# PufferAI/PufferLib

Hardware: NVIDIA H100
Metric: agent-steps/sec (env step + PPO rollout/update hot path) (higher is better)
Workload: dtype f32 (env state int32; policy GEMMs tf32 like the reference)

## Files before the change

pufferlib_b200/csrc/mlp_update.cu:

```cuda
#include <cuda.h>
#include <stdlib.h>

#include "pb_common.cuh"
#include "tma.cuh"
#include "wgmma.cuh"

namespace {

constexpr int TILE_M = 64, HID = 128, FEAT = 128, NO = 8;
constexpr int KBLK = 32;
constexpr int W_KBLK_BYTES = HID * KBLK * 4;
constexpr int X_KBLK_BYTES = TILE_M * KBLK * 4;
constexpr int X_TILE_BYTES = 4 * X_KBLK_BYTES;
constexpr int G_KBLK_BYTES = HID * 32 * 4;
constexpr int NSTAGE = 3;
constexpr int THREADS = 256;
constexpr int SM_W = 0;
constexpr int SM_X = 4 * W_KBLK_BYTES;
constexpr int SM_G = SM_X + NSTAGE * X_TILE_BYTES;
constexpr int SM_WH = SM_G + 2 * G_KBLK_BYTES;
constexpr int SM_BE = SM_WH + NO * HID * 4;
constexpr int SM_OUT = SM_BE + HID * 4;
constexpr int SM_DO = SM_OUT + 2 * TILE_M * NO * 4;
constexpr int SM_RED = SM_DO + TILE_M * NO * 4;
constexpr int SM_BAR = SM_RED + 8 * NO * 4;
constexpr int SMEM_TOTAL = SM_BAR + 64;
constexpr int TAIL = NO * HID + HID + NO;
static_assert(SMEM_TOTAL <= 227 * 1024, "shared memory budget (227 KiB per block on sm_90)");

struct FusedParams {
    const int64_t* actions;
    const float* old_logprobs;
    const float* adv;
    const float* returns;
    const float* old_values;
    const float* adv_norm;
    int64_t row_slab_stride;
    int64_t m;
    int64_t slab_rows;
    int64_t slab_stride_rows;
    int tiles_per_slab, n_tiles;
    int n_act;
    float clip, vclip, vf_coef, ent_coef;
    int clip_vloss;
    float* part_dw;
    float* part_tail;
    double* stats;
    float* dpre_out;
    float* dbg_hidden;
    float* dbg_dpre;
    float* dbg_dout;
    const float* w_heads;
    const float* b_enc;
    const float* b_heads;
};

__device__ __forceinline__ void tma_load_2d(void* dst, const CUtensorMap* map, int c0, int c1, uint64_t* bar) {
    asm volatile(
        "cp.async.bulk.tensor.2d.shared::cluster.global.tile.mbarrier::complete_tx::bytes [%0], [%1, {%2, %3}], [%4];" ::"r"(
            smem_u32(dst)),
        "l"(reinterpret_cast<uint64_t>(map)), "r"(c0), "r"(c1), "r"(smem_u32(bar))
        : "memory");
}

__device__ __forceinline__ uint32_t to_tf32(float x) {
    uint32_t r;
    asm("cvt.rna.tf32.f32 %0, %1;" : "=r"(r) : "f"(x));
    return r;
}

__device__ __forceinline__ void mma_tf32(float (&c)[4], const uint32_t (&a)[4], uint32_t b0, uint32_t b1) {
    asm volatile("mma.sync.aligned.m16n8k8.row.col.f32.tf32.tf32.f32 {%0,%1,%2,%3}, {%4,%5,%6,%7}, {%8,%9}, {%0,%1,%2,%3};"
                 : "+f"(c[0]), "+f"(c[1]), "+f"(c[2]), "+f"(c[3])
                 : "r"(a[0]), "r"(a[1]), "r"(a[2]), "r"(a[3]), "r"(b0), "r"(b1));
}

__device__ __forceinline__ uint32_t g_off(int n, int l) {
    return (uint32_t)((l >> 5) * G_KBLK_BYTES + n * 128 + ((((l & 31) >> 2) ^ (n & 7)) << 4) + (l & 3) * 4);
}
__device__ __forceinline__ uint32_t x_off(int r, int f) {
    return (uint32_t)((f >> 5) * X_KBLK_BYTES + r * 128 + ((((f & 31) >> 2) ^ (r & 7)) << 4) + (f & 3) * 4);
}

struct RowStats { float pg, v, ent, okl, kl, clipped; };

__device__ __forceinline__ RowStats ppo_row_sub(float z_lo, float z_hi, int sub, int lane, const FusedParams& p, int act,
                                                float old_lp, float adv, float ret, float old_v, float& g_lo, float& g_hi) {
    const unsigned full = 0xffffffffu;
    const int n = p.n_act;
    const bool lo_ok = sub < n, hi_ok = sub + 4 < n;
    float mx = fmaxf(lo_ok ? z_lo : -INFINITY, hi_ok ? z_hi : -INFINITY);
    mx = fmaxf(mx, __shfl_xor_sync(full, mx, 1));
    mx = fmaxf(mx, __shfl_xor_sync(full, mx, 2));
    float sum = (lo_ok ? expf(z_lo - mx) : 0.f) + (hi_ok ? expf(z_hi - mx) : 0.f);
    sum += __shfl_xor_sync(full, sum, 1);
    sum += __shfl_xor_sync(full, sum, 2);
    const float lse = mx + logf(sum);
    const float nl_lo = z_lo - lse, nl_hi = z_hi - lse;
    const float pk_lo = lo_ok ? expf(nl_lo) : 0.f, pk_hi = hi_ok ? expf(nl_hi) : 0.f;
    float ent = -(lo_ok ? pk_lo * nl_lo : 0.f) - (hi_ok ? pk_hi * nl_hi : 0.f);
    ent += __shfl_xor_sync(full, ent, 1);
    ent += __shfl_xor_sync(full, ent, 2);
    const int a = act < 0 ? 0 : (act >= n ? n - 1 : act);
    const int base = lane & ~3;
    const float nl_a = __shfl_sync(full, (a >> 2) ? nl_hi : nl_lo, base | (a & 3));
    const float v_new = __shfl_sync(full, (n >> 2) ? z_hi : z_lo, base | (n & 3));
    const float logratio = nl_a - old_lp;
    const float ratio = expf(logratio);
    const float pg1 = -adv * ratio;
    const float rc = fminf(fmaxf(ratio, 1.f - p.clip), 1.f + p.clip);
    const float pg2 = -adv * rc;
    const float pg = fmaxf(pg1, pg2);
    const float in_range = (ratio >= 1.f - p.clip && ratio <= 1.f + p.clip) ? 1.f : 0.f;
    float g_ratio;
    if (pg1 > pg2) g_ratio = -adv;
    else if (pg1 < pg2) g_ratio = -adv * in_range;
    else g_ratio = 0.5f * (-adv) + 0.5f * (-adv * in_range);
    const float inv_m = 1.0f / (float)p.m;
    const float g_nlp = g_ratio * ratio * inv_m;
    const float dv = v_new - ret;
    float vl, g_v;
    if (p.clip_vloss) {
        const float d = v_new - old_v;
        const float dc = fminf(fmaxf(d, -p.vclip), p.vclip);
        const float vc = old_v + dc;
        const float vu = dv * dv, vcl = (vc - ret) * (vc - ret);
        vl = fmaxf(vu, vcl);
        const float v_in = (d >= -p.vclip && d <= p.vclip) ? 1.f : 0.f;
        const float gu = 2.f * dv, gc = 2.f * (vc - ret) * v_in;
        g_v = vu > vcl ? gu : (vu < vcl ? gc : 0.5f * (gu + gc));
    } else {
        vl = dv * dv;
        g_v = 2.f * dv;
    }
    const float gv_out = 0.5f * p.vf_coef * g_v * inv_m;
    const float g_ent = p.ent_coef * inv_m;
    g_lo = lo_ok ? g_nlp * ((sub == a ? 1.f : 0.f) - pk_lo) + g_ent * pk_lo * (nl_lo + ent) : 0.f;
    g_hi = hi_ok ? g_nlp * ((sub + 4 == a ? 1.f : 0.f) - pk_hi) + g_ent * pk_hi * (nl_hi + ent) : 0.f;
    if (sub == n) g_lo = gv_out;
    if (sub + 4 == n) g_hi = gv_out;
    RowStats s;
    s.pg = pg; s.v = vl; s.ent = ent; s.okl = -logratio; s.kl = (ratio - 1.f) - logratio;
    s.clipped = fabsf(ratio - 1.f) > p.clip ? 1.f : 0.f;
    return s;
}

template <bool TF32_EPI, bool DW_KERNEL>
__global__ void __launch_bounds__(THREADS, 1)
k_mlp_update(const __grid_constant__ CUtensorMap map_x, const __grid_constant__ CUtensorMap map_w, const FusedParams p) {
    extern __shared__ __align__(1024) uint8_t smem[];
    uint64_t* w_full = reinterpret_cast<uint64_t*>(smem + SM_BAR);
    uint64_t* x_full = w_full + 1;
    float* wh = reinterpret_cast<float*>(smem + SM_WH);
    const float* be = reinterpret_cast<const float*>(smem + SM_BE);
    float* outp = reinterpret_cast<float*>(smem + SM_OUT);
    float* dos = reinterpret_cast<float*>(smem + SM_DO);
    float* red = reinterpret_cast<float*>(smem + SM_RED);
    uint8_t* gbuf = smem + SM_G;
    const int tid = threadIdx.x, warp = tid >> 5, lane = tid & 31, g = lane >> 2, t = lane & 3;
    const int wg = warp >> 2, wq = warp & 3;
    const int n_my = (p.n_tiles - (int)blockIdx.x + (int)gridDim.x - 1) / (int)gridDim.x;

    auto issue = [&](int it) {
        const int tile = (int)blockIdx.x + it * (int)gridDim.x;
        const int64_t row0 = (int64_t)(tile / p.tiles_per_slab) * p.slab_stride_rows + (int64_t)(tile % p.tiles_per_slab) * TILE_M;
        const int s = it % NSTAGE;
        mbar_expect_tx(&x_full[s], X_TILE_BYTES);
        for (int kb = 0; kb < 4; ++kb)
            tma_load_2d(smem + SM_X + s * X_TILE_BYTES + kb * X_KBLK_BYTES, &map_x, kb * KBLK, (int)row0, &x_full[s]);
    };
    if (tid == 0) {
        mbar_init(w_full, 1);
        for (int s = 0; s < NSTAGE; ++s) mbar_init(&x_full[s], 1);
        mbar_fence_init();
    }
    for (int i = tid; i < NO * HID; i += THREADS) wh[i] = p.w_heads[i];
    if (tid < HID) reinterpret_cast<float*>(smem + SM_BE)[tid] = p.b_enc[tid];
    __syncthreads();
    if (tid == 0) {
        mbar_expect_tx(w_full, 4 * W_KBLK_BYTES);
        for (int kb = 0; kb < 4; ++kb) tma_load_2d(smem + SM_W + kb * W_KBLK_BYTES, &map_w, kb * KBLK, 0, w_full);
        for (int it = 0; it < NSTAGE && it < n_my; ++it) issue(it);
    }

    const int hr0 = 64 * wg + 16 * wq + g, hr1 = hr0 + 8;
    const int lr = tid >> 2, sub = tid & 3;
    const float bh_lo = p.b_heads[sub], bh_hi = p.b_heads[sub + 4];
    uint32_t hb[8][2], ga[4];
    float whr[2][NO];
    if (TF32_EPI) {
        const int hh = warp >> 2;
#pragma unroll
        for (int ks = 0; ks < 8; ++ks) {
            hb[ks][0] = to_tf32(wh[g * HID + 64 * hh + 8 * ks + t]);
            hb[ks][1] = to_tf32(wh[g * HID + 64 * hh + 8 * ks + t + 4]);
        }
        ga[0] = to_tf32(wh[t * HID + hr0]);
        ga[1] = to_tf32(wh[t * HID + hr1]);
        ga[2] = to_tf32(wh[(t + 4) * HID + hr0]);
        ga[3] = to_tf32(wh[(t + 4) * HID + hr1]);
    } else {
#pragma unroll
        for (int a = 0; a < NO; ++a) {
            whr[0][a] = wh[a * HID + hr0];
            whr[1][a] = wh[a * HID + hr1];
        }
    }

    float dwacc[64];
#pragma unroll
    for (int i = 0; i < 64; ++i) dwacc[i] = 0.f;
    float dwh[4] = {0.f, 0.f, 0.f, 0.f};
    float be_acc[2] = {0.f, 0.f};
    float bh_acc[2] = {0.f, 0.f};
    double st[6] = {0, 0, 0, 0, 0, 0};
    const float adv_mean = p.adv_norm ? p.adv_norm[0] : 0.f, adv_rstd = p.adv_norm ? p.adv_norm[1] : 1.f;
    const bool need_old_v = p.clip_vloss || !p.returns;
    const uint32_t w_addr = smem_u32(smem + SM_W), g_addr = smem_u32(gbuf);

    for (int it = 0; it < n_my; ++it) {
        const int s = it % NSTAGE;
        const int tile = (int)blockIdx.x + it * (int)gridDim.x;
        const int slab = tile / p.tiles_per_slab, tis = tile - slab * p.tiles_per_slab;
        const int64_t lrow0 = (int64_t)tis * TILE_M;
        const int rows_left = (int)(p.slab_rows - lrow0 < TILE_M ? p.slab_rows - lrow0 : TILE_M);
        const int64_t i0 = (int64_t)slab * p.slab_rows + lrow0;
        const bool valid = lr < rows_left;
        int act = 0;
        float old_lp = 0.f, adv = 0.f, ret = 0.f, old_v = 0.f;
        if (valid) {
            const int64_t ri = (int64_t)slab * p.row_slab_stride + lrow0 + lr;
            act = (int)p.actions[ri];
            old_lp = p.old_logprobs[ri];
            adv = p.adv[ri];
            if (need_old_v) old_v = p.old_values[ri];
            if (p.returns) ret = p.returns[ri];
        }
        if (it == 0) mbar_wait(w_full, 0);
        mbar_wait(&x_full[s], (uint32_t)((it / NSTAGE) & 1));
        const uint8_t* xs = smem + SM_X + s * X_TILE_BYTES;
        const uint32_t x_addr = smem_u32(xs);

        float h[32];
#pragma unroll
        for (int i = 0; i < 32; ++i) h[i] = 0.f;
        wgmma_fence();
#pragma unroll
        for (int kb = 0; kb < 4; ++kb)
#pragma unroll
            for (int k = 0; k < 4; ++k)
                wgmma_m64n64k8_ss(h, wgmma_desc_sw128(w_addr + kb * W_KBLK_BYTES + wg * 8192 + k * 32),
                                  wgmma_desc_sw128(x_addr + kb * X_KBLK_BYTES + k * 32), (kb | k) ? 1 : 0);
        wgmma_commit();
        wgmma_wait<0>();
        wgmma_fence_acc(h);

        {
            const float b0 = be[hr0], b1 = be[hr1];
#pragma unroll
            for (int j = 0; j < 8; ++j) {
                h[4 * j] = fmaxf(h[4 * j] + b0, 0.f);
                h[4 * j + 1] = fmaxf(h[4 * j + 1] + b0, 0.f);
                h[4 * j + 2] = fmaxf(h[4 * j + 2] + b1, 0.f);
                h[4 * j + 3] = fmaxf(h[4 * j + 3] + b1, 0.f);
                const int l = 8 * j + 2 * t;
                *reinterpret_cast<float2*>(gbuf + g_off(hr0, l)) = make_float2(h[4 * j], h[4 * j + 1]);
                *reinterpret_cast<float2*>(gbuf + g_off(hr1, l)) = make_float2(h[4 * j + 2], h[4 * j + 3]);
                if (p.dbg_hidden) {
#pragma unroll
                    for (int e = 0; e < 4; ++e) {
                        const int le = l + (e & 1), he = (e & 2) ? hr1 : hr0;
                        if (le < rows_left) p.dbg_hidden[(i0 + le) * HID + he] = h[4 * j + e];
                    }
                }
            }
        }
        __syncthreads();

        if (TF32_EPI) {
            const int l0 = 16 * (warp & 3) + g, hh = warp >> 2;
            float c[4] = {0.f, 0.f, 0.f, 0.f};
#pragma unroll
            for (int ks = 0; ks < 8; ++ks) {
                const int n0 = 64 * hh + 8 * ks + t;
                const uint32_t a[4] = {*reinterpret_cast<const uint32_t*>(gbuf + g_off(n0, l0)),
                                       *reinterpret_cast<const uint32_t*>(gbuf + g_off(n0, l0 + 8)),
                                       *reinterpret_cast<const uint32_t*>(gbuf + g_off(n0 + 4, l0)),
                                       *reinterpret_cast<const uint32_t*>(gbuf + g_off(n0 + 4, l0 + 8))};
                mma_tf32(c, a, hb[ks][0], hb[ks][1]);
            }
            *reinterpret_cast<float2*>(outp + (hh * TILE_M + l0) * NO + 2 * t) = make_float2(c[0], c[1]);
            *reinterpret_cast<float2*>(outp + (hh * TILE_M + l0 + 8) * NO + 2 * t) = make_float2(c[2], c[3]);
        } else {
            const int l = tid & (TILE_M - 1), a0 = 2 * (tid >> 6);
            float o0 = 0.f, o1 = 0.f;
            if (a0 <= p.n_act) {
#pragma unroll 8
                for (int n = 0; n < HID; ++n) {
                    const float rh = *reinterpret_cast<const float*>(gbuf + g_off(n, l));
                    o0 = fmaf(rh, wh[a0 * HID + n], o0);
                    o1 = fmaf(rh, wh[(a0 + 1) * HID + n], o1);
                }
            }
            *reinterpret_cast<float2*>(outp + l * NO + a0) = make_float2(o0, o1);
        }
        __syncthreads();

        {
            float z_lo = bh_lo + outp[lr * NO + sub], z_hi = bh_hi + outp[lr * NO + sub + 4];
            if (TF32_EPI) {
                z_lo += outp[(TILE_M + lr) * NO + sub];
                z_hi += outp[(TILE_M + lr) * NO + sub + 4];
            }
            const float r_ = p.returns ? ret : adv + old_v;
            const float a_ = (adv - adv_mean) * adv_rstd;
            float g_lo, g_hi;
            const RowStats rs = ppo_row_sub(z_lo, z_hi, sub, lane, p, act, old_lp, a_, r_, old_v, g_lo, g_hi);
            if (!valid) g_lo = g_hi = 0.f;
            if (valid && sub == 0) {
                st[0] += rs.pg; st[1] += rs.v; st[2] += rs.ent; st[3] += rs.okl; st[4] += rs.kl; st[5] += rs.clipped;
            }
            bh_acc[0] += g_lo;
            bh_acc[1] += g_hi;
            dos[lr * NO + sub] = g_lo;
            dos[lr * NO + sub + 4] = g_hi;
            if (p.dbg_dout && valid) {
                p.dbg_dout[(i0 + lr) * 8 + sub] = g_lo;
                p.dbg_dout[(i0 + lr) * 8 + sub + 4] = g_hi;
            }
        }
        __syncthreads();

        float dp[32];
#pragma unroll
        for (int j = 0; j < 8; ++j) {
            if (TF32_EPI) {
                float c[4] = {0.f, 0.f, 0.f, 0.f};
                mma_tf32(c, ga, __float_as_uint(dos[(8 * j + g) * NO + t]), __float_as_uint(dos[(8 * j + g) * NO + t + 4]));
                dp[4 * j] = c[0]; dp[4 * j + 1] = c[1]; dp[4 * j + 2] = c[2]; dp[4 * j + 3] = c[3];
            } else {
                const int l = 8 * j + 2 * t;
                const float4 d0a = *reinterpret_cast<const float4*>(dos + l * NO), d0b = *reinterpret_cast<const float4*>(dos + l * NO + 4);
                const float4 d1a = *reinterpret_cast<const float4*>(dos + (l + 1) * NO), d1b = *reinterpret_cast<const float4*>(dos + (l + 1) * NO + 4);
                const float d0[8] = {d0a.x, d0a.y, d0a.z, d0a.w, d0b.x, d0b.y, d0b.z, d0b.w};
                const float d1[8] = {d1a.x, d1a.y, d1a.z, d1a.w, d1b.x, d1b.y, d1b.z, d1b.w};
                float s00 = 0.f, s01 = 0.f, s10 = 0.f, s11 = 0.f;
#pragma unroll
                for (int a = 0; a < NO; ++a) {
                    s00 = fmaf(d0[a], whr[0][a], s00);
                    s01 = fmaf(d1[a], whr[0][a], s01);
                    s10 = fmaf(d0[a], whr[1][a], s10);
                    s11 = fmaf(d1[a], whr[1][a], s11);
                }
                dp[4 * j] = s00; dp[4 * j + 1] = s01; dp[4 * j + 2] = s10; dp[4 * j + 3] = s11;
            }
#pragma unroll
            for (int e = 0; e < 4; ++e) dp[4 * j + e] = h[4 * j + e] > 0.f ? dp[4 * j + e] : 0.f;
            be_acc[0] += dp[4 * j] + dp[4 * j + 1];
            be_acc[1] += dp[4 * j + 2] + dp[4 * j + 3];
            const float b0 = dos[(8 * j + 2 * t) * NO + g], b1 = dos[(8 * j + 2 * t + 1) * NO + g];
            if (TF32_EPI) {
                const uint32_t a[4] = {__float_as_uint(h[4 * j]), __float_as_uint(h[4 * j + 2]), __float_as_uint(h[4 * j + 1]),
                                       __float_as_uint(h[4 * j + 3])};
                mma_tf32(dwh, a, __float_as_uint(b0), __float_as_uint(b1));
            } else {
                const uint32_t a[4] = {to_tf32(h[4 * j]), to_tf32(h[4 * j + 2]), to_tf32(h[4 * j + 1]), to_tf32(h[4 * j + 3])};
                mma_tf32(dwh, a, to_tf32(b0), to_tf32(b1));
            }
            const int l = 8 * j + 2 * t;
            if (p.dbg_dpre) {
#pragma unroll
                for (int e = 0; e < 4; ++e) {
                    const int le = l + (e & 1), he = (e & 2) ? hr1 : hr0;
                    if (le < rows_left) p.dbg_dpre[(i0 + le) * HID + he] = dp[4 * j + e];
                }
            }
            if (DW_KERNEL) {
                *reinterpret_cast<uint2*>(gbuf + g_off(hr0, l)) = make_uint2(to_tf32(dp[4 * j]), to_tf32(dp[4 * j + 1]));
                *reinterpret_cast<uint2*>(gbuf + g_off(hr1, l)) = make_uint2(to_tf32(dp[4 * j + 2]), to_tf32(dp[4 * j + 3]));
            } else {
                *reinterpret_cast<float2*>(gbuf + g_off(hr0, l)) = make_float2(dp[4 * j], dp[4 * j + 1]);
                *reinterpret_cast<float2*>(gbuf + g_off(hr1, l)) = make_float2(dp[4 * j + 2], dp[4 * j + 3]);
            }
        }

        if (DW_KERNEL) {
            fence_proxy_async_smem();
            __syncthreads();
            const int f0 = 64 * wg + 16 * wq + g;
            uint32_t xa[8][4];
#pragma unroll
            for (int ks = 0; ks < 8; ++ks) {
                const int r0 = 8 * ks + t;
                xa[ks][0] = to_tf32(*reinterpret_cast<const float*>(xs + x_off(r0, f0)));
                xa[ks][1] = to_tf32(*reinterpret_cast<const float*>(xs + x_off(r0, f0 + 8)));
                xa[ks][2] = to_tf32(*reinterpret_cast<const float*>(xs + x_off(r0 + 4, f0)));
                xa[ks][3] = to_tf32(*reinterpret_cast<const float*>(xs + x_off(r0 + 4, f0 + 8)));
            }
            wgmma_fence();
#pragma unroll
            for (int ks = 0; ks < 8; ++ks)
                wgmma_m64n128k8_rs(dwacc, xa[ks], wgmma_desc_sw128(g_addr + (ks >> 2) * G_KBLK_BYTES + (ks & 3) * 32), 1);
            wgmma_commit();
            wgmma_wait<0>();
            wgmma_fence_acc(dwacc);
#pragma unroll
            for (int ks = 0; ks < 8; ++ks)
#pragma unroll
                for (int i = 0; i < 4; ++i) asm volatile("" : "+r"(xa[ks][i])::"memory");
        } else {
            __syncthreads();
#pragma unroll
            for (int k = 0; k < TILE_M / 8; ++k) {
                const int l = 8 * warp + k;
                if (l < rows_left) {
                    const int n = 4 * lane;
                    const float4 v = make_float4(*reinterpret_cast<const float*>(gbuf + g_off(n, l)),
                                                 *reinterpret_cast<const float*>(gbuf + g_off(n + 1, l)),
                                                 *reinterpret_cast<const float*>(gbuf + g_off(n + 2, l)),
                                                 *reinterpret_cast<const float*>(gbuf + g_off(n + 3, l)));
                    __stcs(reinterpret_cast<float4*>(p.dpre_out + (i0 + l) * HID + n), v);
                }
            }
        }
        __syncthreads();
        if (tid == 0 && it + NSTAGE < n_my) {
            fence_proxy_async_smem();
            issue(it + NSTAGE);
        }
    }

    if (DW_KERNEL) {
        float* pd = p.part_dw + (int64_t)blockIdx.x * FEAT * HID;
        const int f0 = 64 * wg + 16 * wq + g;
#pragma unroll
        for (int j = 0; j < 16; ++j) {
            *reinterpret_cast<float2*>(pd + f0 * HID + 8 * j + 2 * t) = make_float2(dwacc[4 * j], dwacc[4 * j + 1]);
            *reinterpret_cast<float2*>(pd + (f0 + 8) * HID + 8 * j + 2 * t) = make_float2(dwacc[4 * j + 2], dwacc[4 * j + 3]);
        }
    }
    float* pt = p.part_tail + (int64_t)blockIdx.x * TAIL;
    pt[(2 * t) * HID + hr0] = dwh[0];
    pt[(2 * t + 1) * HID + hr0] = dwh[1];
    pt[(2 * t) * HID + hr1] = dwh[2];
    pt[(2 * t + 1) * HID + hr1] = dwh[3];
#pragma unroll
    for (int k = 0; k < 2; ++k) {
        be_acc[k] += __shfl_xor_sync(0xffffffffu, be_acc[k], 1);
        be_acc[k] += __shfl_xor_sync(0xffffffffu, be_acc[k], 2);
    }
    if (t == 0) {
        pt[NO * HID + hr0] = be_acc[0];
        pt[NO * HID + hr1] = be_acc[1];
    }
#pragma unroll
    for (int k = 0; k < 2; ++k)
#pragma unroll
        for (int off = 4; off < 32; off <<= 1) bh_acc[k] += __shfl_xor_sync(0xffffffffu, bh_acc[k], off);
    if (lane < 4) {
        red[warp * NO + lane] = bh_acc[0];
        red[warp * NO + lane + 4] = bh_acc[1];
    }
#pragma unroll
    for (int k = 0; k < 6; ++k) {
        double x = st[k];
#pragma unroll
        for (int off = 16; off > 0; off >>= 1) x += __shfl_xor_sync(0xffffffffu, x, off);
        if (lane == 0) atomicAdd(p.stats + k, x);
    }
    __syncthreads();
    if (tid < NO) {
        float v = 0.f;
        for (int w = 0; w < THREADS / 32; ++w) v += red[w * NO + tid];
        pt[NO * HID + HID + tid] = v;
    }
}

__global__ void __launch_bounds__(256) k_update_reduce(const float* __restrict__ part_dw, const float* __restrict__ part_tail,
                                                       int n_parts, float* __restrict__ gflat, double* __restrict__ sumsq_part) {
    __shared__ float sh[4][64];
    __shared__ double sq[2];
    const int e = blockIdx.x * 64 + (threadIdx.x & 63), grp = threadIdx.x >> 6;
    constexpr int NDW = FEAT * HID;
    float s = 0.f;
    if (e < NDW && !part_dw) {
        if (threadIdx.x == 0) sumsq_part[blockIdx.x] = 0.0;
        return;
    }
    if (e < NDW + TAIL) {
        const float* src = e < NDW ? part_dw + e : part_tail + (e - NDW);
        const int64_t stride = e < NDW ? NDW : TAIL;
#pragma unroll 4
        for (int pidx = grp; pidx < n_parts; pidx += 4) s += src[(int64_t)pidx * stride];
    }
    sh[grp][threadIdx.x & 63] = s;
    __syncthreads();
    if (grp == 0) {
        float tot = 0.f;
        if (e < NDW + TAIL) {
            tot = sh[0][threadIdx.x] + sh[1][threadIdx.x] + sh[2][threadIdx.x] + sh[3][threadIdx.x];
            if (e < NDW) gflat[(e % HID) * FEAT + e / HID] = tot;
            else gflat[e] = tot;
        }
        double d = (double)tot * (double)tot;
#pragma unroll
        for (int off = 16; off > 0; off >>= 1) d += __shfl_xor_sync(0xffffffffu, d, off);
        if ((threadIdx.x & 31) == 0) sq[threadIdx.x >> 5] = d;
    }
    __syncthreads();
    if (threadIdx.x == 0) sumsq_part[blockIdx.x] = sq[0] + sq[1];
}

typedef CUresult (*EncodeTiledFn)(CUtensorMap*, CUtensorMapDataType, cuuint32_t, void*, const cuuint64_t*,
                                  const cuuint64_t*, const cuuint32_t*, const cuuint32_t*, CUtensorMapInterleave,
                                  CUtensorMapSwizzle, CUtensorMapL2promotion, CUtensorMapFloatOOBfill);

int make_map2(EncodeTiledFn fn, CUtensorMap* map, const float* base, int64_t rows, int64_t row_stride_floats, int box_rows) {
    const cuuint64_t dims[2] = {(cuuint64_t)FEAT, (cuuint64_t)rows};
    const cuuint64_t strides[1] = {(cuuint64_t)row_stride_floats * 4};
    const cuuint32_t box[2] = {(cuuint32_t)KBLK, (cuuint32_t)box_rows};
    const cuuint32_t estr[2] = {1, 1};
    const CUresult r = fn(map, CU_TENSOR_MAP_DATA_TYPE_FLOAT32, 2, const_cast<float*>(base), dims, strides, box, estr,
                          CU_TENSOR_MAP_INTERLEAVE_NONE, CU_TENSOR_MAP_SWIZZLE_128B, CU_TENSOR_MAP_L2_PROMOTION_L2_128B,
                          CU_TENSOR_MAP_FLOAT_OOB_FILL_NONE);
    PB_REQUIRE(r == CUDA_SUCCESS, PB_ERR_CUDA, "cuTensorMapEncodeTiled failed: %d", (int)r);
    return PB_OK;
}

int num_sms() { return pb_num_sms(); }

int g_update_variant = 2;

}

extern "C" int pb_mlp_update_set_variant(int32_t variant) {
    PB_REQUIRE(variant == 1 || variant == 2, PB_ERR_INVALID, "pb_mlp_update_set_variant: 1 or 2");
    g_update_variant = variant;
    return PB_OK;
}

constexpr int REDUCE_BLOCKS = (FEAT * HID + TAIL + 63) / 64;

extern "C" size_t pb_mlp_update_sumsq_offset(void) {
    return (((size_t)num_sms() * (FEAT * HID + TAIL) * sizeof(float)) + 15) & ~(size_t)15;
}
extern "C" int32_t pb_mlp_update_sumsq_parts(void) { return REDUCE_BLOCKS; }
extern "C" size_t pb_mlp_update_workspace_bytes(void) {
    return pb_mlp_update_sumsq_offset() + REDUCE_BLOCKS * sizeof(double);
}

extern "C" int pb_mlp_update_fused(const float* x, int64_t ldx, int64_t slab_rows, int64_t slab_stride_rows, int32_t n_slabs,
                                   const float* w_enc, const float* b_enc, const float* w_heads, const float* b_heads,
                                   const int64_t* actions, const float* old_logprobs, const float* advantages,
                                   const float* returns, const float* old_values, const float* adv_norm,
                                   int64_t row_slab_stride, int32_t n_act, float clip_coef,
                                   int32_t clip_vloss, float vf_clip_coef, float vf_coef, float ent_coef, float* grad_flat,
                                   double* stats8, void* workspace, size_t workspace_bytes, float* dpre_out,
                                   float* dbg_hidden, float* dbg_dpre, float* dbg_dout, void* stream) {
    PB_REQUIRE(x && w_enc && b_enc && w_heads && b_heads && actions && old_logprobs && advantages && grad_flat && stats8 &&
                   workspace && (returns || old_values),
               PB_ERR_INVALID, "pb_mlp_update_fused: null pointer");
    PB_REQUIRE(n_slabs == 1 || row_slab_stride >= slab_rows, PB_ERR_INVALID, "pb_mlp_update_fused: row slabs overlap");
    PB_REQUIRE(slab_rows >= 1 && n_slabs >= 1 && n_act >= 1 && n_act <= 7 && (!clip_vloss || old_values), PB_ERR_INVALID,
               "pb_mlp_update_fused: bad sizes (slab_rows %lld, n_slabs %d, n_act %d)", (long long)slab_rows, n_slabs, n_act);
    PB_REQUIRE(ldx >= FEAT && ldx % 4 == 0 && ((uintptr_t)x & 15) == 0 && ((uintptr_t)w_enc & 15) == 0, PB_ERR_INVALID,
               "pb_mlp_update_fused: x / w_enc must be 16-byte aligned, ldx a multiple of 4 floats");
    PB_REQUIRE(n_slabs == 1 || slab_stride_rows >= slab_rows, PB_ERR_INVALID, "pb_mlp_update_fused: slabs overlap");
    PB_REQUIRE(workspace_bytes >= pb_mlp_update_workspace_bytes(), PB_ERR_INVALID, "pb_mlp_update_fused: workspace too small");
    PB_REQUIRE(!dbg_hidden || dbg_dpre, PB_ERR_INVALID, "pb_mlp_update_fused: dbg_hidden needs dbg_dpre");
    void* fn = nullptr;
    cudaDriverEntryPointQueryResult qr;
    PB_REQUIRE(cudaGetDriverEntryPoint("cuTensorMapEncodeTiled", &fn, cudaEnableDefault, &qr) == cudaSuccess && fn &&
                   qr == cudaDriverEntryPointSuccess,
               PB_ERR_CUDA, "cuTensorMapEncodeTiled entry point not available");
    const int64_t tiles_per_slab = (slab_rows + TILE_M - 1) / TILE_M;
    const int64_t n_tiles = tiles_per_slab * n_slabs;
    const int64_t map_rows = (int64_t)(n_slabs - 1) * slab_stride_rows + slab_rows;
    PB_REQUIRE(n_tiles <= 0x7FFFFFFF && map_rows <= 0x7FFFFFFF, PB_ERR_UNSUPPORTED, "pb_mlp_update_fused: too many rows");
    alignas(64) CUtensorMap map_x, map_w;
    int rc = make_map2((EncodeTiledFn)fn, &map_x, x, map_rows, ldx, TILE_M);
    if (rc == PB_OK) rc = make_map2((EncodeTiledFn)fn, &map_w, w_enc, HID, FEAT, HID);
    if (rc != PB_OK) return rc;
    cudaStream_t s = (cudaStream_t)stream;
    const int grid = n_tiles < num_sms() ? (int)n_tiles : num_sms();
    FusedParams p;
    p.actions = actions; p.old_logprobs = old_logprobs; p.adv = advantages; p.returns = returns; p.old_values = old_values;
    p.adv_norm = adv_norm; p.row_slab_stride = n_slabs > 1 ? row_slab_stride : slab_rows;
    p.m = slab_rows * n_slabs; p.slab_rows = slab_rows; p.slab_stride_rows = n_slabs > 1 ? slab_stride_rows : slab_rows;
    p.tiles_per_slab = (int)tiles_per_slab; p.n_tiles = (int)n_tiles; p.n_act = n_act;
    p.clip = clip_coef; p.vclip = vf_clip_coef; p.vf_coef = vf_coef; p.ent_coef = ent_coef; p.clip_vloss = clip_vloss;
    p.part_dw = (float*)workspace; p.part_tail = (float*)workspace + (size_t)num_sms() * FEAT * HID;
    p.w_heads = w_heads; p.b_enc = b_enc; p.b_heads = b_heads;
    p.stats = stats8; p.dpre_out = dpre_out; p.dbg_hidden = dbg_hidden; p.dbg_dpre = dbg_dpre; p.dbg_dout = dbg_dout;
    PB_CUDA(cudaMemsetAsync(stats8, 0, 8 * sizeof(double), s));
    static bool attr_set = false;
    if (!attr_set) {
        PB_CUDA(cudaFuncSetAttribute(k_mlp_update<false, false>, cudaFuncAttributeMaxDynamicSharedMemorySize, SMEM_TOTAL));
        PB_CUDA(cudaFuncSetAttribute(k_mlp_update<false, true>, cudaFuncAttributeMaxDynamicSharedMemorySize, SMEM_TOTAL));
        PB_CUDA(cudaFuncSetAttribute(k_mlp_update<true, true>, cudaFuncAttributeMaxDynamicSharedMemorySize, SMEM_TOTAL));
        attr_set = true;
    }
    if (dpre_out) k_mlp_update<false, false><<<grid, THREADS, SMEM_TOTAL, s>>>(map_x, map_w, p);
    else if (g_update_variant == 2) k_mlp_update<true, true><<<grid, THREADS, SMEM_TOTAL, s>>>(map_x, map_w, p);
    else k_mlp_update<false, true><<<grid, THREADS, SMEM_TOTAL, s>>>(map_x, map_w, p);
    PB_LAUNCH_CHECK();
    k_update_reduce<<<REDUCE_BLOCKS, 256, 0, s>>>(dpre_out ? nullptr : p.part_dw, p.part_tail, grid, grad_flat,
                                                  reinterpret_cast<double*>((char*)workspace + pb_mlp_update_sumsq_offset()));
    PB_LAUNCH_CHECK();
    return PB_OK;
}
```

Before: 405.6 million.

## Defer dW wgmma into next tile's forward GEMM via double-buffered gradient smem

The dW accumulation wgmma for tile it is now issued asynchronously during tile it+1, right after the forward GEMM commit, so it overlaps with the bias/ReLU/epilogue work. To make this safe the gradient staging buffer is double-buffered, and the X pipeline drops from 3 to 2 stages to free shared memory. The xa register fragments now live across iterations, which raises register pressure. The shallower TMA prefetch could also expose load latency. A final drain after the loop issues the last tile's dW.

```diff
diff --git a/pufferlib_b200/csrc/mlp_update.cu b/pufferlib_b200/csrc/mlp_update.cu
--- a/pufferlib_b200/csrc/mlp_update.cu
+++ b/pufferlib_b200/csrc/mlp_update.cu
@@ -13,12 +13,13 @@
 constexpr int X_KBLK_BYTES = TILE_M * KBLK * 4;
 constexpr int X_TILE_BYTES = 4 * X_KBLK_BYTES;
 constexpr int G_KBLK_BYTES = HID * 32 * 4;
-constexpr int NSTAGE = 3;
+constexpr int NSTAGE = 2;
 constexpr int THREADS = 256;
 constexpr int SM_W = 0;
 constexpr int SM_X = 4 * W_KBLK_BYTES;
+constexpr int G_BYTES = 2 * G_KBLK_BYTES;
 constexpr int SM_G = SM_X + NSTAGE * X_TILE_BYTES;
-constexpr int SM_WH = SM_G + 2 * G_KBLK_BYTES;
+constexpr int SM_WH = SM_G + 2 * G_BYTES;
 constexpr int SM_BE = SM_WH + NO * HID * 4;
 constexpr int SM_OUT = SM_BE + HID * 4;
 constexpr int SM_DO = SM_OUT + 2 * TILE_M * NO * 4;
@@ -217,6 +218,13 @@
     const float adv_mean = p.adv_norm ? p.adv_norm[0] : 0.f, adv_rstd = p.adv_norm ? p.adv_norm[1] : 1.f;
     const bool need_old_v = p.clip_vloss || !p.returns;
     const uint32_t w_addr = smem_u32(smem + SM_W), g_addr = smem_u32(gbuf);
+    uint32_t xa[8][4];
+    auto dw_issue = [&](uint32_t (&a)[8][4], uint32_t gaddr) {
+#pragma unroll
+        for (int ks = 0; ks < 8; ++ks)
+            wgmma_m64n128k8_rs(dwacc, a[ks], wgmma_desc_sw128(gaddr + (ks >> 2) * G_KBLK_BYTES + (ks & 3) * 32), 1);
+        wgmma_commit();
+    };
 
     for (int it = 0; it < n_my; ++it) {
         const int s = it % NSTAGE;
@@ -240,6 +248,7 @@
         mbar_wait(&x_full[s], (uint32_t)((it / NSTAGE) & 1));
         const uint8_t* xs = smem + SM_X + s * X_TILE_BYTES;
         const uint32_t x_addr = smem_u32(xs);
+        uint8_t* gb = gbuf + (DW_KERNEL ? (it & 1) * G_BYTES : 0);
 
         float h[32];
 #pragma unroll
@@ -252,7 +261,12 @@
                 wgmma_m64n64k8_ss(h, wgmma_desc_sw128(w_addr + kb * W_KBLK_BYTES + wg * 8192 + k * 32),
                                   wgmma_desc_sw128(x_addr + kb * X_KBLK_BYTES + k * 32), (kb | k) ? 1 : 0);
         wgmma_commit();
-        wgmma_wait<0>();
+        if (DW_KERNEL && it > 0) {
+            dw_issue(xa, g_addr + ((it - 1) & 1) * G_BYTES);
+            wgmma_wait<1>();
+        } else {
+            wgmma_wait<0>();
+        }
         wgmma_fence_acc(h);
 
         {
@@ -264,8 +278,8 @@
                 h[4 * j + 2] = fmaxf(h[4 * j + 2] + b1, 0.f);
                 h[4 * j + 3] = fmaxf(h[4 * j + 3] + b1, 0.f);
                 const int l = 8 * j + 2 * t;
-                *reinterpret_cast<float2*>(gbuf + g_off(hr0, l)) = make_float2(h[4 * j], h[4 * j + 1]);
-                *reinterpret_cast<float2*>(gbuf + g_off(hr1, l)) = make_float2(h[4 * j + 2], h[4 * j + 3]);
+                *reinterpret_cast<float2*>(gb + g_off(hr0, l)) = make_float2(h[4 * j], h[4 * j + 1]);
+                *reinterpret_cast<float2*>(gb + g_off(hr1, l)) = make_float2(h[4 * j + 2], h[4 * j + 3]);
                 if (p.dbg_hidden) {
 #pragma unroll
                     for (int e = 0; e < 4; ++e) {
@@ -283,10 +297,10 @@
 #pragma unroll
             for (int ks = 0; ks < 8; ++ks) {
                 const int n0 = 64 * hh + 8 * ks + t;
-                const uint32_t a[4] = {*reinterpret_cast<const uint32_t*>(gbuf + g_off(n0, l0)),
-                                       *reinterpret_cast<const uint32_t*>(gbuf + g_off(n0, l0 + 8)),
-                                       *reinterpret_cast<const uint32_t*>(gbuf + g_off(n0 + 4, l0)),
-                                       *reinterpret_cast<const uint32_t*>(gbuf + g_off(n0 + 4, l0 + 8))};
+                const uint32_t a[4] = {*reinterpret_cast<const uint32_t*>(gb + g_off(n0, l0)),
+                                       *reinterpret_cast<const uint32_t*>(gb + g_off(n0, l0 + 8)),
+                                       *reinterpret_cast<const uint32_t*>(gb + g_off(n0 + 4, l0)),
+                                       *reinterpret_cast<const uint32_t*>(gb + g_off(n0 + 4, l0 + 8))};
                 mma_tf32(c, a, hb[ks][0], hb[ks][1]);
             }
             *reinterpret_cast<float2*>(outp + (hh * TILE_M + l0) * NO + 2 * t) = make_float2(c[0], c[1]);
@@ -297,7 +311,7 @@
             if (a0 <= p.n_act) {
 #pragma unroll 8
                 for (int n = 0; n < HID; ++n) {
-                    const float rh = *reinterpret_cast<const float*>(gbuf + g_off(n, l));
+                    const float rh = *reinterpret_cast<const float*>(gb + g_off(n, l));
                     o0 = fmaf(rh, wh[a0 * HID + n], o0);
                     o1 = fmaf(rh, wh[(a0 + 1) * HID + n], o1);
                 }
@@ -376,19 +390,26 @@
                 }
             }
             if (DW_KERNEL) {
-                *reinterpret_cast<uint2*>(gbuf + g_off(hr0, l)) = make_uint2(to_tf32(dp[4 * j]), to_tf32(dp[4 * j + 1]));
-                *reinterpret_cast<uint2*>(gbuf + g_off(hr1, l)) = make_uint2(to_tf32(dp[4 * j + 2]), to_tf32(dp[4 * j + 3]));
+                *reinterpret_cast<uint2*>(gb + g_off(hr0, l)) = make_uint2(to_tf32(dp[4 * j]), to_tf32(dp[4 * j + 1]));
+                *reinterpret_cast<uint2*>(gb + g_off(hr1, l)) = make_uint2(to_tf32(dp[4 * j + 2]), to_tf32(dp[4 * j + 3]));
             } else {
-                *reinterpret_cast<float2*>(gbuf + g_off(hr0, l)) = make_float2(dp[4 * j], dp[4 * j + 1]);
-                *reinterpret_cast<float2*>(gbuf + g_off(hr1, l)) = make_float2(dp[4 * j + 2], dp[4 * j + 3]);
+                *reinterpret_cast<float2*>(gb + g_off(hr0, l)) = make_float2(dp[4 * j], dp[4 * j + 1]);
+                *reinterpret_cast<float2*>(gb + g_off(hr1, l)) = make_float2(dp[4 * j + 2], dp[4 * j + 3]);
             }
         }
 
         if (DW_KERNEL) {
             fence_proxy_async_smem();
             __syncthreads();
+            if (it > 0) {
+                wgmma_wait<0>();
+                wgmma_fence_acc(dwacc);
+#pragma unroll
+                for (int ks = 0; ks < 8; ++ks)
+#pragma unroll
+                    for (int i = 0; i < 4; ++i) asm volatile("" : "+r"(xa[ks][i])::"memory");
+            }
             const int f0 = 64 * wg + 16 * wq + g;
-            uint32_t xa[8][4];
 #pragma unroll
             for (int ks = 0; ks < 8; ++ks) {
                 const int r0 = 8 * ks + t;
@@ -397,17 +418,6 @@
                 xa[ks][2] = to_tf32(*reinterpret_cast<const float*>(xs + x_off(r0 + 4, f0)));
                 xa[ks][3] = to_tf32(*reinterpret_cast<const float*>(xs + x_off(r0 + 4, f0 + 8)));
             }
-            wgmma_fence();
-#pragma unroll
-            for (int ks = 0; ks < 8; ++ks)
-                wgmma_m64n128k8_rs(dwacc, xa[ks], wgmma_desc_sw128(g_addr + (ks >> 2) * G_KBLK_BYTES + (ks & 3) * 32), 1);
-            wgmma_commit();
-            wgmma_wait<0>();
-            wgmma_fence_acc(dwacc);
-#pragma unroll
-            for (int ks = 0; ks < 8; ++ks)
-#pragma unroll
-                for (int i = 0; i < 4; ++i) asm volatile("" : "+r"(xa[ks][i])::"memory");
         } else {
             __syncthreads();
 #pragma unroll
@@ -415,10 +425,10 @@
                 const int l = 8 * warp + k;
                 if (l < rows_left) {
                     const int n = 4 * lane;
-                    const float4 v = make_float4(*reinterpret_cast<const float*>(gbuf + g_off(n, l)),
-                                                 *reinterpret_cast<const float*>(gbuf + g_off(n + 1, l)),
-                                                 *reinterpret_cast<const float*>(gbuf + g_off(n + 2, l)),
-                                                 *reinterpret_cast<const float*>(gbuf + g_off(n + 3, l)));
+                    const float4 v = make_float4(*reinterpret_cast<const float*>(gb + g_off(n, l)),
+                                                 *reinterpret_cast<const float*>(gb + g_off(n + 1, l)),
+                                                 *reinterpret_cast<const float*>(gb + g_off(n + 2, l)),
+                                                 *reinterpret_cast<const float*>(gb + g_off(n + 3, l)));
                     __stcs(reinterpret_cast<float4*>(p.dpre_out + (i0 + l) * HID + n), v);
                 }
             }
@@ -431,6 +441,14 @@
     }
 
     if (DW_KERNEL) {
+        wgmma_fence();
+        dw_issue(xa, g_addr + ((n_my - 1) & 1) * G_BYTES);
+        wgmma_wait<0>();
+        wgmma_fence_acc(dwacc);
+#pragma unroll
+        for (int ks = 0; ks < 8; ++ks)
+#pragma unroll
+            for (int i = 0; i < 4; ++i) asm volatile("" : "+r"(xa[ks][i])::"memory");
         float* pd = p.part_dw + (int64_t)blockIdx.x * FEAT * HID;
         const int f0 = 64 * wg + 16 * wq + g;
 #pragma unroll
```

Measured after the change: 427.9 million, median of 6. +5.5%, better.
